# yabebalFantaye/MCEvidence

Hardware: AMD Instinct MI355X
Metric: knn_queries_per_sec (higher is better)
Workload: dtype f16 filter + f64 refine (exact f64 results)

## Files before the change

### mcevidence_amd/csrc/capi_search.hpp

```cpp
#pragma once
namespace {

double ln_unit_ball(int d) { return 0.5 * d * std::log(M_PI) - std::lgamma(1.0 + 0.5 * d); }

hipError_t launch_sym_merge(int KCAP, double* pd, int* pi, int64_t nq_pad, const mce::SymParams& sym, int qb_lo, int qb_hi, hipStream_t st, int stride = 1)
{
    const int nb = qb_hi > qb_lo ? (qb_hi - qb_lo + stride - 1) / stride : 0;
    if (nb <= 0) return hipSuccess;
    const dim3 g((unsigned)nb), b(mce::kSymMergeThreads);
    static_assert(mce::kSymMergeThreads == mce::f16_qpb(4), "one merge block per query block");
    switch (KCAP) {
        case 4: hipLaunchKernelGGL(mce::sym_merge_kernel<4>, g, b, 0, st, pd, pi, nq_pad, sym.bucket_cnt, sym.bucket_flag, sym.bucket, sym.cap, qb_lo, stride); break;
        case 8: hipLaunchKernelGGL(mce::sym_merge_kernel<8>, g, b, 0, st, pd, pi, nq_pad, sym.bucket_cnt, sym.bucket_flag, sym.bucket, sym.cap, qb_lo, stride); break;
        case 12: hipLaunchKernelGGL(mce::sym_merge_kernel<12>, g, b, 0, st, pd, pi, nq_pad, sym.bucket_cnt, sym.bucket_flag, sym.bucket, sym.cap, qb_lo, stride); break;
        default: hipLaunchKernelGGL(mce::sym_merge_kernel<16>, g, b, 0, st, pd, pi, nq_pad, sym.bucket_cnt, sym.bucket_flag, sym.bucket, sym.cap, qb_lo, stride); break;
    }
    return hipGetLastError();
}

struct KernelBracket {
    bool on = false; hipStream_t st = nullptr;
    hipError_t begin() const
    {
        if (!on) return hipSuccess;
// ... 307 lines not shown
        units = mce::panel_unit_count(g);
        for (int u = 0; g_prof_on && u < units; ++u) {
            int pp, aa, lo, hi;
            mce::panel_unit_decode(u, g, pp, aa);
            mce::panel_unit_tiles(pp, aa, g, lo, hi);
            tiles += hi - lo;
        }
    } else {
        const double tpb = mce::kHWaves * mce::kHQT, T = (double)((nr + 31) / 32);
        for (int b = 0; b < p.nqblk; ++b) tiles += std::min(tpb * (b + 1), T);
    }
    g_last_flops_main = tiles * 16.0 * 1024.0 * 32.0 * p.KST;
    return units;
}

int Search::symmetric()
{
    char* const sw = ws + p.off_sym;
    mce::KnnF16Args a = sym_args(p, ws, nr, d, K, self_exclude);
    const Tuning tun = read_tuning();
    const int seed_rows = tun.sym_seed_rows > 0 ? tun.sym_seed_rows : (p.KST == 1 ? 65536 : 32768) * (p.apo && p.nparts >= 4 ? 2 : 1);
    const int seed_share = tun.sym_seed_share;
    auto sym_seed_for = [&](int kk) {
        int cfg = mce::f16_seed_cfg(p.nchunk, p.CT, kk + a.self_exclude, seed_rows, seed_share, MCE_H_SEED_TG);
        for (int tg = MCE_H_SEED_TG / 2; cfg == 0 && tg >= 1; tg /= 2)
            cfg = mce::f16_seed_cfg(p.nchunk, p.CT, kk + a.self_exclude, seed_rows, seed_share, tg);
        if (cfg) cfg |= ((tun.sym_seed_mode >= 0 ? tun.sym_seed_mode : kSymSeedMode[p.KST]) & 3) << 28;
        return cfg;
    };
    const int qb_lo = p.nparts > 1 && !p.apo ? (int)((int64_t)p.nqblk * p.part / p.nparts) : 0;
    const int qb_hi = p.nparts > 1 && !p.apo ? (int)((int64_t)p.nqblk * (p.part + 1) / p.nparts) : p.nqblk;
    p.sym_qb_lo = qb_lo; p.sym_qb_hi = qb_hi;
    const bool panel_kernel = !tun.sym_kernel_f16 || p.nparts > 1 || p.twopass;
    mce::PanelGeom geom;
    geom.qb_lo = qb_lo; geom.qb_hi = qb_hi; geom.tpb = mce::kHWaves * mce::kHQT; geom.ct = p.CT; geom.tpp = a.sym.panel * p.CT; geom.sym_on = 1;
    geom.ntiles = (int)((nr + 31) / 32) + (int)(((nr + 31) / 32) & 1);
    const bool apo = p.apo && p.nparts > 1 && !p.twopass && panel_kernel;
    const bool chains1 = !apo && p.nparts == 1 && panel_kernel && !p.twopass && p.sym_nsplit > 1;
    if (apo) { geom.blk_first = p.part; geom.blk_stride = p.nparts; }
    if (apo || chains1) {
        const int pn = apo ? p.apo_panel : p.sym_panel;
        if (pn > 0 && (apo || tun.sym_panel <= 0)) { a.sym.panel = pn; geom.tpp = a.sym.panel * p.CT; }
        geom.nsplit = std::max(1, apo ? p.apo_nsplit : p.sym_nsplit);
        if (geom.nsplit > 1) {
            a.sym.done = reinterpret_cast<int*>(sw + p.sl.keys_b);
            MCE_HIP(mce::zero_async(a.sym.done, (size_t)p.nqblk * geom.nsplit * sizeof(int), st));
            if (!apo) {
                hipLaunchKernelGGL(mce::sym_chain_init_kernel, dim3((unsigned)p.nqblk), dim3(512), 0, st, pd, pi, p.nq_pad, p.KCAP, geom.nsplit, 0, 1);
                MCE_HIP(hipGetLastError());
            }
        }
    }
    const bool unit_table = apo || geom.nsplit > 1;
    const int npass = p.twopass ? 2 : 1;
    int seed_used = 0;
    for (int pass = 0; pass < npass; ++pass) {
        const bool lower = pass == 1;
        const int Kp = !p.twopass ? K : (lower ? K - 16 : 16);
        double* const pdp = pd + (lower ? list_set(p, 1) : 0);
        int* const pip = pi + (lower ? list_set(p, 1) : 0);
        if (lower) {
            MCE_HIP(mce::zero_async(a.sym.bucket_cnt, (size_t)3 * p.nqblk * sizeof(int), st));
            a.sym.slot_stride = p.KCAP;
        }
        a.ksel = lower ? K : Kp;
        a.seed_cfg = sym_seed_for(a.ksel);
        a.part_d = pdp; a.part_i = pip;
        a.qblk0 = qb_lo;
        a.nqblk_run = qb_hi - qb_lo;
        if (apo) {
            a.qblk0 = p.part; a.qblk_stride = p.nparts; a.nqblk_run = mce::apo_rank_count(p.nqblk, p.part, p.nparts);
        }
        if (a.nqblk_run > 0 && phase != 2) MCE_HIP((lower ? p.vh->launch_sym_pre32 : p.vh->launch_sym_pre)(a, st));
        a.qblk0 = 0; a.qblk_stride = 1; a.nqblk_run = 0;
        if (phase == 1) return MCE_OK;
        if (pass == 0) seed_used = a.seed_cfg;
        a.seed_cfg = 0;
        a.ksel = Kp;
        a.lo_d = lower ? pd : nullptr; a.lo_i = lower ? pi : nullptr;
        if (pass == 0) MCE_HIP(kb.begin());
        if (panel_kernel) {
            mce::PanelArgs pa;
            pa.Yh = static_cast<const _Float16*>(a.Yh); pa.Xh = static_cast<const _Float16*>(a.Xh); pa.qinfo = a.qinfo; pa.params = a.params;
            pa.X = a.X; pa.Y = a.Y; pa.rperm = a.rperm;
            pa.part_d = pdp; pa.part_i = pip; pa.nq = nq; pa.nr = nr; pa.nq_pad = p.nq_pad; pa.self_offset = 0;
            pa.D = d; pa.ksel = Kp; pa.self_exclude = a.self_exclude; pa.spin_limit = tun.spin_limit;
            pa.sym = a.sym; pa.debug = tun.panel_debug; pa.geom = geom; pa.lo_d = a.lo_d; pa.lo_i = a.lo_i;
            if (unit_table) {
                const int nun = mce::panel_unit_count(geom);
                if ((size_t)nun * sizeof(mce::PanelUnit) > (size_t)p.nq_pad * sizeof(int)) return fail(MCE_ERR_INVALID, "symmetric sweep: %d units do not fit the table", nun);
                mce::PanelUnit* tab = reinterpret_cast<mce::PanelUnit*>(sw + p.sl.vals_a);
                if (nun > 0) {
                    hipLaunchKernelGGL(mce::panel_unit_table_kernel, dim3((unsigned)((nun + 255) / 256)), dim3(256), 0, st, geom, nun, tab);
                    MCE_HIP(hipGetLastError());
                }
                pa.units = tab;
            }
            MCE_HIP((lower ? p.vh->launch_panel_lower : p.vh->launch_panel)(pa, st));
        } else {
            MCE_HIP(p.vh->launch_sym(a, st));
        }
        if (pass == 0) MCE_HIP(kb.end());
        if (apo) break;
        MCE_HIP((lower ? p.vh->launch_sym_repair_lower : p.vh->launch_sym_repair)(a, st));
        if (geom.nsplit > 1) {
            hipLaunchKernelGGL(mce::sym_chain_clear_kernel, dim3((unsigned)p.nqblk), dim3(512), 0, st, a.sym.bucket_flag, pdp, pip, p.nq_pad, p.KCAP, geom.nsplit, 0, 1);
            MCE_HIP(hipGetLastError());
        }
        MCE_HIP(launch_sym_merge(p.KCAP, pdp, pip, p.nq_pad, a.sym, qb_lo, qb_hi, st));
    }
    p.sym_active = true;
    p.L = geom.nsplit > 1 ? geom.nsplit : npass;
    const int sym_units = sym_units_and_flops(p, geom, panel_kernel, nr, a.sym.panel);
    g_last_flops_all = g_last_flops_main + (double)(seed_used & 0xffff) * p.CT * (double)(qb_hi - qb_lo) * 16.0 * 1024.0 * 32.0 * p.KST;
    snprintf(g_last_kernel, sizeof(g_last_kernel), "%s symmetric%s%s%s grid=%d block=%d lds=%zu qt=%d ct=%d panel=%d seed=%dx%d/%d bucket=%d", p.vh->name, panel_kernel ? " panel-kernel" : "",
             p.twopass ? " two passes" : "", geom.blk_stride > 1 ? " pairs-once" : (geom.nsplit > 1 ? " chains" : ""), sym_units,
             mce::kHThreads, panel_kernel ? p.vh->lds_bytes_panel : p.vh->lds_bytes_sym, p.QT, p.CT, a.sym.panel, seed_used & 0xffff, (seed_used >> 16) & 0xfff, (seed_used >> 28) & 3, p.sl.cap);
    return MCE_OK;
}

int Search::f16_sweep(const F16Search& f)
{
    mce::KnnF16Args a = f16_args(p, ws, f.sX, nq, f.sY, nr, d, K, self_exclude, self_offset);
    auto seed_cfg = [&](int ksel) { return sweep_seed_cfg(p.nchunk / p.rsplit, p.CT, ksel + a.self_exclude); };
    MCE_HIP(kb.begin());
    if (p.twopass) {
        a.ksel = 16;
        a.seed_cfg = seed_cfg(16);
        MCE_HIP(p.vh->launch(a, st));
        a.lo_d = pd; a.lo_i = pi;
        a.part_d = pd + list_set(p, p.rsplit); a.part_i = pi + list_set(p, p.rsplit);
        a.ksel = K - 16;
        a.seed_cfg = 0;
        MCE_HIP(p.vh->launch_lower(a, st));
    } else {
        a.seed_cfg = seed_cfg(K);
        if (p.wide_ok) MCE_HIP(p.vh->launch_wide(a, st));
        else MCE_HIP(p.vh->launch(a, st));
    }
    MCE_HIP(kb.end());
    const int seed_first = p.twopass ? seed_cfg(16) : a.seed_cfg;
    g_last_flops_main = (double)p.nqblk * ((double)p.nchunk + (double)(seed_first & 0xffff) * p.rsplit) * p.CT * 16.0 * 1024.0 * 32.0 * p.KST +
                        (p.twopass ? (double)p.nqblk * (double)p.nchunk * p.CT * 16.0 * 1024.0 * 32.0 * p.KST : 0.0);
    g_last_flops_all = g_last_flops_main;
    char seed_txt[48] = "";
    if (seed_first) snprintf(seed_txt, sizeof(seed_txt), " seed=%dx%d", seed_first & 0xffff, seed_first >> 16);
    const bool wide = p.wide_ok && !p.twopass;
    snprintf(g_last_kernel, sizeof(g_last_kernel), "%s grid=%d block=%d lds=%zu qt=%d ct=%d rsplit=%d%s%s%s", p.vh->name,
             (wide ? p.nqblk / 2 : p.nqblk) * p.rsplit, mce::kHThreads, wide ? p.vh->lds_bytes_wide : p.vh->lds_bytes, wide ? 2 * p.QT : p.QT, p.CT, p.rsplit,
             p.twopass ? " two passes" : "", seed_txt, wide ? " wide" : "");
    return MCE_OK;
}

int Search::fp64()
{
    const int threads = 256;
    double* yf = reinterpret_cast<double*>(ws + p.off_yf);
    hipLaunchKernelGGL(mce::pack_refs_kernel, dim3((unsigned)((p.nrow_pad + threads - 1) / threads)), dim3(threads), 0, st, dY, nr,
                       (int)d, p.KS, p.nrow_pad, center, yf);
    MCE_HIP(hipGetLastError());
    mce::KnnArgs a;
    a.Yf = yf; a.nchunk_total = p.nchunk; a.rsplit = p.rsplit; a.X = dX; a.center = center; a.nq = nq; a.D = d;
    a.nq_pad = p.nq_pad; a.nqblk = p.nqblk; a.self_exclude = self_exclude; a.self_offset = self_offset;
    a.ksel = p.ksel > K ? p.ksel : K;
    a.part_d = pd; a.part_i = pi;
    MCE_HIP(kb.begin());
    MCE_HIP(p.v->launch(a, st));
// ... 98 lines not shown
```

### mcevidence_amd/csrc/knn_panel.hpp

```cpp
#pragma once
#include "knn_f16.hpp"

namespace mce {

struct PanelArgs {
    const _Float16* Yh;
    const _Float16* Xh;
    const double* qinfo;
    const double* params;
    const double* X;
    const double* Y;
    const int* rperm;
    double* part_d;
    int* part_i;
    int64_t nq, nr, nq_pad, self_offset;
    int D, ksel, self_exclude, spin_limit;
    int debug;
    SymParams sym;
    PanelGeom geom;
    const PanelUnit* units = nullptr;
    const double* lo_d = nullptr;
    const int* lo_i = nullptr;
};

#ifndef MCE_PANEL_STATS
#define MCE_PANEL_STATS 0
#endif
#ifndef MCE_PANEL_NPASS
#define MCE_PANEL_NPASS 3
#endif
#ifndef MCE_PANEL_STAGE_KB
#define MCE_PANEL_STAGE_KB MCE_H_STAGE_KB
#endif
#ifndef MCE_PANEL_QUEUE
#define MCE_PANEL_QUEUE MCE_H_QUEUE
#endif
#ifndef MCE_PANEL_TRIGGER
#define MCE_PANEL_TRIGGER 192
#endif
#ifndef MCE_PANEL_ABL
#define MCE_PANEL_ABL 0
#endif

__host__ __device__ constexpr int panel_chunk_tiles(int KST) { return MCE_PANEL_STAGE_KB / KST / 2 * 2; }
constexpr int kPanelQueue = MCE_PANEL_QUEUE;
__host__ __device__ constexpr size_t panel_lds_bytes(int KST)
{
    return (size_t)2 * panel_chunk_tiles(KST) * KST * 1024
           + (size_t)kHWaves * kPanelQueue * 16
           + (size_t)kHWaves * kHQT * 32 * 4 + 128
           + (size_t)kHWaves * kHQT * 32 * 4
           + (size_t)kHWaves * panel_chunk_tiles(KST) * kHQT * 4;
}

template <class T> __device__ __forceinline__ const __attribute__((address_space(1))) T* gptr(const T* p)
{
    return (const __attribute__((address_space(1))) T*)p;
}
template <class T> __device__ __forceinline__ __attribute__((address_space(1))) T* gptr_w(T* p)
{
    return (__attribute__((address_space(1))) T*)p;
}

__device__ __forceinline__ float vmaxf(float a, float b)
{
    float r;
    asm("v_max_f32 %0, %1, %2" : "=v"(r) : "v"(a), "v"(b));
    return r;
}

template <int KST, int KCAP, bool LOWER = false>
__global__ __launch_bounds__(kHThreads, 2) void knn_panel_kernel(PanelArgs args_by_value)
{
    static_assert(kHQT == 2 && kHNL == 1, "8 waves x 2 query tiles, one list per owner lane");
    constexpr int QT = 2;
    constexpr int QPW = 64;
    constexpr int QPB = kHWaves * QPW;
    constexpr int TPB = QPB / 32;
    constexpr int CT = panel_chunk_tiles(KST);
    constexpr int CHUNK_BYTES = CT * KST * 1024;
    constexpr int VPT = CHUNK_BYTES / 16 / kHThreads;
    static_assert(CHUNK_BYTES % (16 * kHThreads) == 0 && CT % 2 == 0, "chunk geometry");
    constexpr int QN = kPanelQueue;
    (void)args_by_value;
// ... 100 lines not shown
            } else if (lane == 0) {
                gptr_w(a->sym.bucket_flag)[qblk] = 1;
            }
        }
    }

    v8h b[QT][KST];
    float G[QT], cR[QT];
    unsigned lanew[QT];
    const int k_last = MCE_ARGS()->ksel - 1;
    {
        const ArgsPtr a = MCE_ARGS();
        const auto Xh = gptr(a->Xh);
#pragma unroll
        for (int qt = 0; qt < QT; ++qt) {
            const int64_t q = qwave0 + qt * 32 + (lane & 31);
#pragma unroll
            for (int ks = 0; ks < KST; ++ks)
                b[qt][ks] = *(const __attribute__((address_space(1))) v8h*)(Xh + q * (int64_t)(16 * KST) + 16 * ks + 8 * (lane >> 5));
            lanew[qt] = ((unsigned)(qt * 32 + (lane & 31)) << kHRelBits) | (unsigned)(4 * (lane >> 5));
            cR[qt] = -__builtin_huge_valf();
            G[qt] = -__builtin_huge_valf();
        }
    }
    double gq_a[QT], gq_c[QT], own_a = 0.0, s2c, rowc;
    {
        const ArgsPtr a = MCE_ARGS();
        const auto params = gptr(a->params);
        const auto qinfo = gptr(a->qinfo);
        const double p_scale = params[HP_SCALE], p_ey = params[HP_EY], p_ym = params[HP_YHATMAX], p_rho = params[HP_RHO];
        s2c = p_scale * p_scale;
        rowc = f16_row_const(p_ym);
#pragma unroll
        for (int qt = 0; qt < QT; ++qt) {
            const int64_t q = qwave0 + qt * 32 + (lane & 31);
            gq_a[qt] = 0.0;
            gq_c[qt] = -INF;
            if (q < a->nq && MCE_PANEL_ABL != 1) {
                const F16GateTerms t = f16_gate_terms(qinfo[2 * q], qinfo[2 * q + 1], p_ey, p_ym, p_rho, KST);
                gq_a[qt] = t.a;
                gq_c[qt] = t.c;
            }
        }
        {
            const int64_t q = qwave0 + lane;
            if (q < a->nq) own_a = f16_gate_a(qinfo[2 * q], p_ey, KST);
        }
    }
    auto gate_of = [&](double thr, int qt) __attribute__((always_inline)) -> float { return f16_gate(thr, s2c, gq_a[qt], gq_c[qt]); };
    auto own_row_gate = [&](double thr) __attribute__((always_inline)) -> float { return f16_row_gate(thr, s2c, own_a, rowc); };
    {
        const ArgsPtr a = MCE_ARGS();
        const int64_t q = qwave0 + lane;
        double t0 = INF;
        if (sym_on) t0 = __longlong_as_double((long long)__hip_atomic_load(gptr(a->sym.thr) + q, __ATOMIC_RELAXED, __HIP_MEMORY_SCOPE_AGENT));
        else if (a->sym.thr) t0 = __longlong_as_double((long long)gptr(a->sym.thr)[q]);
        seed_thr = t0;
        double tl = own_d[KCAP - 1];
#pragma unroll
        for (int k = 0; k < KCAP - 1; ++k) tl = (k == k_last) ? own_d[k] : tl;
        t0 = fmin(t0, tl);
        sthr[lane] = __double2float_ru(t0);
#pragma unroll
        for (int qt = 0; qt < QT; ++qt) G[qt] = gate_of(__shfl(t0, qt * 32 + (lane & 31), 64), qt);
        if (sym_on) {
#pragma unroll
            for (int qt = 0; qt < QT; ++qt) cR[qt] = gq_c[qt] > -INF ? f16_round_up(gq_c[qt]) : -__builtin_huge_valf();
        }
    }

    const int dbg_flags = MCE_ARGS()->debug;
    const int qlimit_gate = (dbg_flags & 8) ? -1 : QN - 64;
    int qcount = 0;
    int nredo = 0;

    auto drain = [&]() __attribute__((always_inline)) {
#if MCE_PANEL_STATS
        const long long t_d0 = clock64();
        st_drains += 1; st_enq += qcount;
#endif
        const ArgsPtr a = MCE_ARGS();
        const auto X = gptr(a->X);
        const auto Y = gptr(a->Y);
        const int D = a->D;
        const int64_t nq = a->nq, nr = a->nr;
        const int self_exclude = a->self_exclude;
        const int64_t self_offset = a->self_offset;
        const auto rperm = gptr(a->rperm);
        {
            const int sub = lane & 7;
            constexpr int NPASS = KST > 2 ? 1 : MCE_PANEL_NPASS;
            constexpr int EPL = KST > 2 ? 8 : 4;
            for (int b0 = 0; b0 < qcount; b0 += NPASS * 8) {
                int qlp[NPASS], ep[NPASS];
                bool okp[NPASS];
                const __attribute__((address_space(1))) double* xp[NPASS];
                const __attribute__((address_space(1))) double* yp[NPASS];
#pragma unroll
                for (int u = 0; u < NPASS; ++u) {
                    const int e = b0 + u * 8 + (lane >> 3);
                    ep[u] = e;
                    int ql = 0, j = 0;
                    const bool valid = e < qcount;
                    if (valid) {
                        const unsigned ent = (unsigned)wq[e];
                        ql = (int)(ent >> kHRelBits);
                        j = (int)(ent & ((1u << kHSymRowBits) - 1u));
                    }
                    qlp[u] = ql;
                    const int64_t q = qwave0 + ql;
                    okp[u] = valid && j < nr && q < nq && !(self_exclude && (int64_t)j == self_offset + q);
                    xp[u] = X + (okp[u] ? q : 0) * (int64_t)D;
                    yp[u] = Y + (okp[u] ? (int64_t)j : 0) * D;
                }
                double xv[NPASS][EPL], yv[NPASS][EPL];
#pragma unroll
                for (int u = 0; u < NPASS; ++u)
#pragma unroll
                    for (int v = 0; v < EPL; ++v) {
                        const int iv = (sub + 8 * v < D) ? sub + 8 * v : (sub < D ? sub : D - 1);
                        xv[u][v] = xp[u][iv];
                        yv[u][v] = yp[u][iv];
                    }
#pragma unroll
                for (int u = 0; u < NPASS; ++u) {
                    double a0 = 0.0;
#pragma unroll
                    for (int v = 0; v < EPL; ++v) {
                        const double t = (sub + 8 * v < D) ? xv[u][v] - yv[u][v] : 0.0;
                        a0 = fma(t, t, a0);
                    }
                    a0 += __shfl_xor(a0, 1, 64);
                    a0 += __shfl_xor(a0, 2, 64);
                    a0 += __shfl_xor(a0, 4, 64);
                    if (sub == 0 && ep[u] < qcount) {
                        wqd[ep[u]] = okp[u] ? a0 : -1.0;
                        bool col = okp[u] && !(a0 > (double)sthr[qlp[u]]);
                        if constexpr (LOWER) {
                            if (col) {
                                const int64_t o = (int64_t)(KCAP - 1) * a->nq_pad + qwave0 + qlp[u];
                                const double ld = gptr(a->lo_d)[o];
                                const int li = gptr(a->lo_i)[o];
                                const int jr = (int)((unsigned)wq[ep[u]] & ((1u << kHSymRowBits) - 1u));
                                const int jc = rperm ? rperm[jr] : jr;
                                col = a0 > ld || (a0 == ld && jc > li);
                            }
                        }
                        if (col) wnx[ep[u]] = atomicExch(&whead[qlp[u]], ep[u]);
                    }
                }
            }
        }
        __builtin_amdgcn_fence(__ATOMIC_ACQ_REL, "wavefront");
#if MCE_PANEL_STATS
        const long long t_dA = clock64();
        st_tA += t_dA - t_d0;
#endif
        {
            const auto sp_thr = gptr_w(a->sym.thr);
            const auto sp_rrow = gptr_w(a->sym.rrow);
            const auto sp_rtile = gptr_w(a->sym.rtile);
            const auto sp_slots = gptr_w(a->sym.slots);
            const auto sp_bucket_cnt = gptr_w(a->sym.bucket_cnt);
            const auto sp_bucket_flag = gptr_w(a->sym.bucket_flag);
            const auto sp_bucket = gptr_w(a->sym.bucket);
            const int sp_cap = a->sym.cap;
            const int ksel = a->ksel;
            auto row_gate = [&](double thr, int row) { return f16_row_gate_of(thr, gptr(a->qinfo)[2 * (int64_t)row], a->params, KST); };
            for (int e0 = 0; e0 < qcount; e0 += 64) {
                const int e = e0 + lane;
                const bool valid = e < qcount;
                const unsigned ent = valid ? (unsigned)wq[e] : 0u;
                const int ql = (int)(ent >> kHRelBits);
                const int j = (int)(ent & ((1u << kHSymRowBits) - 1u));
                const bool rowflag = (ent >> kHSymRowBits) & 1u;
                const double d2 = valid ? wqd[e] : -1.0;
                const bool ok = valid && d2 >= 0.0;
                const int oj = ok ? (rperm ? rperm[j] : j) : -1;
                bool rs = ok && rowflag;
                if (rs) {
                    const int jb = j / QPB;
                    rs = d2 <= __longlong_as_double((long long)__hip_atomic_load(sp_thr + j, __ATOMIC_RELAXED, __HIP_MEMORY_SCOPE_AGENT));
                    if constexpr (LOWER) {
                        if (rs) {
                            const int64_t o = (int64_t)(KCAP - 1) * a->nq_pad + j;
                            const double ld = gptr(a->lo_d)[o];
                            const int li = gptr(a->lo_i)[o];
                            const int sc = rperm ? rperm[qwave0 + ql] : (int)(qwave0 + ql);
                            rs = d2 > ld || (d2 == ld && sc > li);
                        }
                    }
                    if (rs) rs = sym_slot_insert<KCAP>(sp_slots, sp_thr, sp_rrow, sp_rtile, ksel, j, d2, row_gate);
                    if (rs) {
                        const int slot = __hip_atomic_fetch_add(sp_bucket_cnt + jb, 1, __ATOMIC_RELAXED, __HIP_MEMORY_SCOPE_AGENT);
                        if ((unsigned)slot < (unsigned)sp_cap) {
                            const auto en = sp_bucket + ((int64_t)jb * sp_cap + slot);
                            en->d2 = d2;
                            en->src = rperm ? rperm[qwave0 + ql] : (int)(qwave0 + ql);
                            en->row = j;
                        } else {
                            sp_bucket_flag[jb] = 1;
                        }
                    }
                }
                if (valid) wq[e] = oj;
            }
        }
        __builtin_amdgcn_fence(__ATOMIC_ACQ_REL, "wavefront");
#if MCE_PANEL_STATS
        const long long t_dR = clock64();
        st_tR += t_dR - t_dA;
#endif
        {
            int cur = whead[lane];
            whead[lane] = -1;
            while (__any(cur >= 0)) {
                const bool on = cur >= 0;
                const int ce = on ? cur : 0;
                const double d2 = on ? wqd[ce] : INF;
                const int j = wq[ce];
                cur = on ? wnx[ce] : -1;
                list_insert<KCAP>(own_d, own_i, d2, j);
            }
        }
        qcount = 0;
        double thr_own = own_d[KCAP - 1];
#pragma unroll
        for (int k = 0; k < KCAP - 1; ++k) thr_own = (k == k_last) ? own_d[k] : thr_own;
        thr_own = fmin(thr_own, seed_thr);
        if (sym_on) {
            const auto sp_thr = gptr_w(a->sym.thr);
            const auto sp_rrow = gptr_w(a->sym.rrow);
            const auto sp_rtile = gptr_w(a->sym.rtile);
            const int64_t q = qwave0 + lane;
            double t = thr_own;
            float R = 0.0f;
            if (q < nq) {
                if (t < INF) {
                    const unsigned long long mb = (unsigned long long)__double_as_longlong(t);
                    const unsigned rb = __float_as_uint(own_row_gate(t));
                    const unsigned long long ob = __hip_atomic_fetch_min(sp_thr + q, mb, __ATOMIC_RELAXED, __HIP_MEMORY_SCOPE_AGENT);
                    const unsigned orb = __hip_atomic_fetch_min(sp_rrow + q, rb, __ATOMIC_RELAXED, __HIP_MEMORY_SCOPE_AGENT);
                    t = fmin(t, __longlong_as_double((long long)ob));
                    R = __uint_as_float(rb < orb ? rb : orb);
                } else {
                    t = __longlong_as_double((long long)__hip_atomic_load(sp_thr + q, __ATOMIC_RELAXED, __HIP_MEMORY_SCOPE_AGENT));
                    const unsigned rb = __float_as_uint(own_row_gate(t));
                    const unsigned orb = __hip_atomic_fetch_min(sp_rrow + q, rb, __ATOMIC_RELAXED, __HIP_MEMORY_SCOPE_AGENT);
                    R = __uint_as_float(rb < orb ? rb : orb);
                }
            }
            thr_own = t;
            seed_thr = t;
            float m = R;
#pragma unroll
            for (int o = 16; o >= 1; o >>= 1) m = fmaxf(m, __shfl_xor(m, o, 64));
            if ((lane & 31) == 0) __hip_atomic_store(sp_rtile + ((qwave0 + lane) >> 5), m, __ATOMIC_RELAXED, __HIP_MEMORY_SCOPE_AGENT);
        }
        sthr[lane] = __double2float_ru(thr_own);
#pragma unroll
        for (int qt = 0; qt < QT; ++qt) G[qt] = gate_of(__shfl(thr_own, qt * 32 + (lane & 31), 64), qt);
#if MCE_PANEL_STATS
        st_tD += clock64() - t_d0;
#endif
    };

    auto event = [&](const v16f& c, const float (&l1)[5], const int qt, const float gq, const bool rowflag, const int jb0, const unsigned todo, const int qlimit) __attribute__((always_inline)) -> unsigned {
        return f16_event<true>(c, l1, lanew[qt], gq, rowflag, jb0, todo, qlimit, wq, qcount);
    };

    const auto Yh_bytes = (const __attribute__((address_space(1))) char*)MCE_ARGS()->Yh;
    auto stage_async = [&](int64_t c, int buf) { f16_stage_chunk<VPT>(Yh_bytes + c * (int64_t)CHUNK_BYTES, stage0 + buf * CHUNK_BYTES, tid, wave); };
    auto load_a = [&](const char* lp, v8h (&a)[KST]) { f16_load_a<KST>(lp, a); };
    auto mfma_first = [&](const v8h (&a)[KST], v16f (&acc)[QT]) __attribute__((always_inline)) {
#pragma unroll
        for (int qt = 0; qt < QT; ++qt) {
            v16f z = {0.f, 0.f, 0.f, 0.f, 0.f, 0.f, 0.f, 0.f, 0.f, 0.f, 0.f, 0.f, 0.f, 0.f, 0.f, 0.f};
            acc[qt] = __builtin_amdgcn_mfma_f32_32x32x16_f16(a[0], b[qt][0], z, 0, 0, 0);
        }
    };
    auto mfma_rest = [&](const v8h (&a)[KST], v16f (&acc)[QT]) __attribute__((always_inline)) {
#pragma unroll
        for (int ks = 1; ks < KST; ++ks)
#pragma unroll
            for (int qt = 0; qt < QT; ++qt) acc[qt] = __builtin_amdgcn_mfma_f32_32x32x16_f16(a[ks], b[qt][ks], acc[qt], 0, 0, 0);
    };
#if defined(__HIP_DEVICE_COMPILE__)
#define MCE_ORDER(GATED_, NEXT_) asm volatile("" : "+v"(GATED_[0]), "+v"(GATED_[1]), "+v"(NEXT_[0]), "+v"(NEXT_[1]))
// ... 188 lines not shown
```

### mcevidence_amd/csrc/prune.hip

```cpp
#include "prune.hpp"
#include "zero_fill.hpp"

#include <cstdlib>
#include <cstring>

#include <rocprim/device/device_radix_sort.hpp>

#include <algorithm>

namespace mce {

namespace {

constexpr int kThreads = 256;

size_t align_up(size_t x, size_t a) { return (x + a - 1) / a * a; }

constexpr int kCoordBits = 24;
constexpr int kMinCoordBits32 = 18;
constexpr int kAlign = 64;
constexpr int kAlignLevels = 6;

int top_tree_levels(int64_t n_units)
{
    const int64_t groups = (n_units + kAlign - 1) / kAlign;
    int L = 0;
    while (((int64_t)1 << L) < groups) ++L;
    return L;
}

template <class Key>
__global__ __launch_bounds__(kThreads) void kd_key_kernel(const int* __restrict__ perm_in, int64_t n, int64_t n_pad, int unit_rows,
                                                          int n_units, int top_levels, int level, const float* __restrict__ Cf, int d, int dim,
                                                          int cbits, Key* __restrict__ keys, int* __restrict__ vals, int64_t pos0 = 0, int64_t pos1 = -1)
{
    const int64_t pos = pos0 + (int64_t)blockIdx.x * kThreads + threadIdx.x;
    if (pos >= (pos1 < 0 ? n_pad : pos1)) return;
    const int row = perm_in ? perm_in[pos] : (pos < n ? (int)pos : -1);
    const int u = (int)(pos / unit_rows);
    const int cu = u / kAlign;
    int clo = 0, chi = (n_units + kAlign - 1) / kAlign;
    unsigned id = 0;
    int l = 0;
    for (; l < level && l < top_levels; ++l) {
        if (chi - clo > 1) {
            const int mid = (clo + chi) >> 1;
            if (cu < mid) { chi = mid; id = 2 * id; }
            else { clo = mid; id = 2 * id + 1; }
        } else {
            id = 2 * id;
        }
    }
    for (int half = kAlign >> 1; l < level; ++l, half >>= 1) id = 2 * id + ((u & half) ? 1u : 0u);
    unsigned b = 0xFFFFFFFFu;
    if (row >= 0) {
        const float c = Cf[(int64_t)dim * n + row];
        b = __float_as_uint(c);
        b = (b & 0x80000000u) ? ~b : (b | 0x80000000u);
        if (b == 0xFFFFFFFFu) b = 0xFFFFFFFEu;
        b >>= (32 - cbits);
        if (b == (0xFFFFFFFFu >> (32 - cbits))) b -= 1u;
    } else {
        b >>= (32 - cbits);
    }
    keys[pos] = (Key)(((Key)id << cbits) | (Key)b);
    vals[pos] = row;
}

constexpr int kGroupRows = kAlign * kPruneTileRows;
constexpr int kBottomSlots = kGroupRows + kGroupRows / 32;
__device__ __forceinline__ int bslot(int i) { return i + (i >> 5); }
__global__ __launch_bounds__(kThreads) void kd_bottom_kernel(int* __restrict__ perm, int64_t n, int64_t n_pad, int top_levels, const float* __restrict__ Cf, int d,
                                                             int64_t group0 = 0)
{
    static_assert(kGroupRows == 8 * kThreads, "eight slots per thread");
    __shared__ unsigned long long key[kBottomSlots];
    __shared__ int val[2][kGroupRows];
    const int64_t base = (group0 + (int64_t)blockIdx.x) * kGroupRows;
    const int m = (int)(n_pad - base < kGroupRows ? n_pad - base : kGroupRows);
    for (int i = threadIdx.x; i < kGroupRows; i += kThreads) val[0][i] = i < m ? perm[base + i] : -2;
    __syncthreads();
    int cur = 0;
    for (int l = 0; l < kAlignLevels; ++l) {
        const int dim = (top_levels + l) % d;
// ... 485 lines not shown
    hipLaunchKernelGGL(group_box_kernel, blocks_for((int64_t)nqblk * d), dim3(kThreads), 0, st, out.tbox_q, same_set ? ntile_r : ntile_q, d,
                       qpb / kPruneTileRows, nqblk, box_q);
    if ((e = hipGetLastError()) != hipSuccess) return e;
    static_assert(kBandKeys % kThreads == 0 && kPruneMaxDim * 2 <= kThreads, "chunk_list_kernel geometry");
    if (nchunk <= kListStage) {
        static bool attr_set[16] = {};
        int dev = 0;
        (void)hipGetDevice(&dev);
        if (dev >= 16 || !attr_set[dev]) {
            e = hipFuncSetAttribute(reinterpret_cast<const void*>(chunk_list_kernel), hipFuncAttributeMaxDynamicSharedMemorySize, (int)chunk_list_lds_bytes(kListStage));
            if (e != hipSuccess) return e;
            if (dev < 16) attr_set[dev] = true;
        }
        hipLaunchKernelGGL(chunk_list_kernel, dim3((unsigned)nqblk), dim3(kThreads), chunk_list_lds_bytes((int)nchunk), st, box_q, box_r, (int)nchunk, d, list_d_b, list_c_b);
    } else {
        hipLaunchKernelGGL(chunk_list_big_kernel, dim3((unsigned)nqblk), dim3(kThreads), 0, st, box_q, box_r, (int)nchunk, d, list_d_b, list_c_b);
    }
    if ((e = hipGetLastError()) != hipSuccess) return e;
    {
        float* bkey_a = reinterpret_cast<float*>(ws + L.bkey_a);
        float* bkey_b = reinterpret_cast<float*>(ws + L.bkey_b);
        int* bval_a = reinterpret_cast<int*>(ws + L.bval_a);
        int* border = reinterpret_cast<int*>(ws + L.border);
        const int nwaves = nqblk * kPruneWavesPerBlock;
        const int tpw = qpb / kPruneTileRows / kPruneWavesPerBlock;
        hipLaunchKernelGGL(wave_cost_kernel, dim3((unsigned)((nwaves + kThreads - 1) / kThreads)), dim3(kThreads), 0, st, out.tbox_q, nwaves, tpw,
                           same_set ? ntile_r : ntile_q, d, bkey_a, bval_a);
        if ((e = hipGetLastError()) != hipSuccess) return e;
        size_t tb2 = L.tmp_bytes;
        e = rocprim::radix_sort_pairs_desc(tmp, tb2, (const float*)bkey_a, bkey_b, (const int*)bval_a, border, (size_t)nwaves, 0u, 32u, st);
        if (e != hipSuccess) return e;
        out.border = border;
    }
    out.Ys = Ys;
    out.rperm = perm_r;
    out.clist = list_c_b;
    out.cdist = list_d_b;
    return hipSuccess;
}

namespace {

constexpr int kNormRows = 256;
__global__ __launch_bounds__(kNormRows) void norm_key_kernel(const double* __restrict__ Y, int64_t n, int64_t n_pad, int d,
                                                             const double* __restrict__ center, unsigned* __restrict__ keys,
                                                             int* __restrict__ vals)
{
    extern __shared__ double tile[];
    const int64_t r0 = (int64_t)blockIdx.x * kNormRows;
    const int64_t rows = n - r0 < kNormRows ? (n - r0 > 0 ? n - r0 : 0) : kNormRows;
    const int ld = d + 1;
    for (int64_t e = threadIdx.x; e < rows * d; e += kNormRows) {
        const int r = (int)(e / d), c = (int)(e - (int64_t)r * d);
        tile[r * ld + c] = Y[r0 * d + e] - center[c];
    }
    __syncthreads();
    const int64_t pos = r0 + threadIdx.x;
    if (pos >= n_pad) return;
    unsigned k = 0xFFFFFFFFu;
    if (pos < n) {
        double s = 0.0;
        for (int i = 0; i < d; ++i) {
            const double t = tile[threadIdx.x * ld + i];
            s = fma(t, t, s);
        }
        k = __float_as_uint((float)s);
        if (k > 0xFFFFFFFEu || s != s) k = 0xFFFFFFFEu;
    }
    keys[pos] = k;
    vals[pos] = pos < n ? (int)pos : -1;
}

}

int sym_layout(int64_t n, int64_t n_pad, int nqblk, int d, int kcap, int qpb, int per_row, SymLayout& L)
{
    size_t off = 0;
    auto take = [&](size_t bytes) { const size_t o = off; off = align_up(off + bytes, 256); return o; };
    L.perm = take((size_t)n_pad * 4);
    L.keys_a = take((size_t)n_pad * 4);
    L.keys_b = take((size_t)n_pad * 4);
    L.vals_a = take((size_t)n_pad * 4);
    L.Ys = take((size_t)n * d * 8);
    L.thr = take((size_t)n_pad * 8);
    L.rrow = take((size_t)n_pad * 4);
    L.rtile = take((size_t)(n_pad / 32) * 4);
    L.slots = take((size_t)n_pad * kcap * 8);
    L.bucket_cnt = take((size_t)nqblk * 4 * 3);
    L.bucket_flag = L.bucket_cnt + (size_t)nqblk * 4;
    L.done = L.bucket_flag + (size_t)nqblk * 4;
    L.cap = per_row * qpb;
    L.bucket = take((size_t)nqblk * L.cap * 16);
    L.tmp_bytes = sort_pairs_tmp_bytes<unsigned>(n_pad, 32u);
    L.tmp = take(L.tmp_bytes);
    L.total = off;
    return 0;
}

hipError_t sym_prepare(const double* dY, int64_t n, int d, const double* center, int64_t n_pad, char* ws, const SymLayout& L, hipStream_t st)
{
    int* perm = reinterpret_cast<int*>(ws + L.perm);
    unsigned* keys_a = reinterpret_cast<unsigned*>(ws + L.keys_a);
    unsigned* keys_b = reinterpret_cast<unsigned*>(ws + L.keys_b);
    int* vals_a = reinterpret_cast<int*>(ws + L.vals_a);
    double* Ys = reinterpret_cast<double*>(ws + L.Ys);
    const unsigned blocks = (unsigned)((n_pad + kNormRows - 1) / kNormRows);
    hipLaunchKernelGGL(norm_key_kernel, dim3(blocks), dim3(kNormRows), (size_t)kNormRows * (d + 1) * sizeof(double), st, dY, n, n_pad, d, center,
                       keys_a, vals_a);
    hipError_t e = hipGetLastError();
    if (e != hipSuccess) return e;
    e = sort_pairs(ws + L.tmp, L.tmp_bytes, (const unsigned*)keys_a, keys_b, (const int*)vals_a, perm, n_pad, 32u, st);
    if (e != hipSuccess) return e;
    hipLaunchKernelGGL(gather_rows_kernel, dim3((unsigned)((n * d + kThreads - 1) / kThreads)), dim3(kThreads), 0, st, dY, perm, n, d, Ys);
    if ((e = hipGetLastError()) != hipSuccess) return e;
    e = zero_async(ws + L.bucket_cnt, (size_t)3 * (L.bucket_flag - L.bucket_cnt), st);
    return e;
}

}
```

### mcevidence_amd/csrc/prune.hpp

```cpp
#pragma once
#include <hip/hip_runtime.h>
#include <stddef.h>
#include <stdint.h>

namespace mce {

constexpr int kPruneTileRows = 32;
constexpr int kPruneMaxDim = 15;
constexpr int64_t kPruneMaxPairs = (int64_t)1 << 30;
constexpr int kPruneWavesPerBlock = 8;

struct PruneLayout {
    size_t perm_r = 0, perm_q = 0;
    size_t keys_a = 0, keys_b = 0;
    size_t vals_b = 0;
    size_t Ys = 0, Xs = 0;
    size_t cf32 = 0;
    size_t tbox_r = 0, tbox_q = 0;
    size_t tboxT_r = 0;
    size_t box_r = 0, box_q = 0;
    size_t bkey_a = 0, bkey_b = 0, bval_a = 0, border = 0;
    size_t list_d_b = 0, list_c_b = 0;
    size_t tmp = 0, tmp_bytes = 0;
    size_t total = 0;
};

int prune_layout(int64_t nq, int64_t nq_pad, int nqblk, int64_t nr, int64_t nr_pad, int64_t nchunk, int d, PruneLayout& L);

constexpr int kPruneBandMantissa = 5;
__host__ __device__ inline float prune_band_floor(float d2)
{
#if defined(__HIP_DEVICE_COMPILE__)
    return __uint_as_float(__float_as_uint(d2) & ~((1u << (23 - kPruneBandMantissa)) - 1u));
#else
    union { float f; unsigned u; } v; v.f = d2; v.u &= ~((1u << (23 - kPruneBandMantissa)) - 1u); return v.f;
#endif
}

struct PruneOut {
    const double* Xs = nullptr;
    const double* Ys = nullptr;
    const int* qperm = nullptr;
    const int* rperm = nullptr;
    const int* clist = nullptr;
    const float* cdist = nullptr;
    const float* tbox_r = nullptr;
    const float* tbox_q = nullptr;
    const float* cbox_r = nullptr;
    const int* border = nullptr;
};

hipError_t prune_prepare(const double* dX, int64_t nq, const double* dY, int64_t nr, int d, bool same_set, int qpb,
                         int chunk_rows, int64_t nq_pad, int nqblk, int64_t nr_pad, int64_t nchunk, char* ws,
                         const PruneLayout& L, hipStream_t st, PruneOut& out, bool perm_ready = false);
hipError_t prune_prepare_part(const double* dY, int64_t nr, int d, int64_t nr_pad, char* ws, const PruneLayout& L, int part, int nparts,
                              hipStream_t st, int64_t& seg_lo, int64_t& seg_hi);

struct SymLayout {
    size_t perm = 0;
    size_t keys_a = 0, keys_b = 0;
    size_t vals_a = 0;
    size_t Ys = 0;
    size_t thr = 0;
    size_t rrow = 0;
    size_t rtile = 0;
    size_t slots = 0;
    size_t bucket_cnt = 0, bucket_flag = 0, done = 0;
    size_t bucket = 0;
    size_t tmp = 0, tmp_bytes = 0;
    size_t total = 0;
    int cap = 0;
};
int sym_layout(int64_t n, int64_t n_pad, int nqblk, int d, int kcap, int qpb, int per_row, SymLayout& L);
hipError_t sym_prepare(const double* dY, int64_t n, int d, const double* center, int64_t n_pad, char* ws, const SymLayout& L,
                       hipStream_t st);

}
```

Before: 26.86 million.

## Refine from padded lane-interleaved f64 image and batch survivor threshold loads

Measured after the change: 27.06 million, median of 6. Within noise of the previous version (+0.8%).

```diff
diff --git a/mcevidence_amd/csrc/capi_search.hpp b/mcevidence_amd/csrc/capi_search.hpp
--- a/mcevidence_amd/csrc/capi_search.hpp
+++ b/mcevidence_amd/csrc/capi_search.hpp
@@ -413,7 +413,8 @@
         if (panel_kernel) {
             mce::PanelArgs pa;
             pa.Yh = static_cast<const _Float16*>(a.Yh); pa.Xh = static_cast<const _Float16*>(a.Xh); pa.qinfo = a.qinfo; pa.params = a.params;
-            pa.X = a.X; pa.Y = a.Y; pa.rperm = a.rperm;
+            if (p.sl.img_pitch != mce::refine_pitch(p.KST)) return fail(MCE_ERR_INVALID, "symmetric sweep: refine image of pitch %d, the kernel reads %d", p.sl.img_pitch, mce::refine_pitch(p.KST));
+            pa.X = pa.Y = reinterpret_cast<const double*>(sw + p.sl.Yimg); pa.rperm = a.rperm;
             pa.part_d = pdp; pa.part_i = pip; pa.nq = nq; pa.nr = nr; pa.nq_pad = p.nq_pad; pa.self_offset = 0;
             pa.D = d; pa.ksel = Kp; pa.self_exclude = a.self_exclude; pa.spin_limit = tun.spin_limit;
             pa.sym = a.sym; pa.debug = tun.panel_debug; pa.geom = geom; pa.lo_d = a.lo_d; pa.lo_i = a.lo_i;
diff --git a/mcevidence_amd/csrc/knn_panel.hpp b/mcevidence_amd/csrc/knn_panel.hpp
--- a/mcevidence_amd/csrc/knn_panel.hpp
+++ b/mcevidence_amd/csrc/knn_panel.hpp
@@ -1,5 +1,6 @@
 #pragma once
 #include "knn_f16.hpp"
+#include "refine_image.hpp"
 
 namespace mce {
 
@@ -266,23 +267,30 @@
         const ArgsPtr a = MCE_ARGS();
         const auto X = gptr(a->X);
         const auto Y = gptr(a->Y);
-        const int D = a->D;
         const int64_t nq = a->nq, nr = a->nr;
         const int self_exclude = a->self_exclude;
         const int64_t self_offset = a->self_offset;
         const auto rperm = gptr(a->rperm);
+        int dl = lane;
+#if defined(__HIP_DEVICE_COMPILE__)
+        asm volatile("" : "+v"(dl));
+#endif
         {
-            const int sub = lane & 7;
+            typedef double v2d __attribute__((ext_vector_type(2)));
+            typedef const __attribute__((address_space(1))) v2d* RowPtr;
+            const int sub = dl & 7;
             constexpr int NPASS = KST > 2 ? 1 : MCE_PANEL_NPASS;
-            constexpr int EPL = KST > 2 ? 8 : 4;
+            constexpr int EPL = refine_epl(KST);
+            constexpr int PITCH = refine_pitch(KST);
+            const auto Xl = X + EPL * sub;
+            const auto Yl = Y + EPL * sub;
             for (int b0 = 0; b0 < qcount; b0 += NPASS * 8) {
                 int qlp[NPASS], ep[NPASS];
                 bool okp[NPASS];
-                const __attribute__((address_space(1))) double* xp[NPASS];
-                const __attribute__((address_space(1))) double* yp[NPASS];
+                RowPtr xp[NPASS], yp[NPASS];
 #pragma unroll
                 for (int u = 0; u < NPASS; ++u) {
-                    const int e = b0 + u * 8 + (lane >> 3);
+                    const int e = b0 + u * 8 + (dl >> 3);
                     ep[u] = e;
                     int ql = 0, j = 0;
                     const bool valid = e < qcount;
@@ -294,24 +302,24 @@
                     qlp[u] = ql;
                     const int64_t q = qwave0 + ql;
                     okp[u] = valid && j < nr && q < nq && !(self_exclude && (int64_t)j == self_offset + q);
-                    xp[u] = X + (okp[u] ? q : 0) * (int64_t)D;
-                    yp[u] = Y + (okp[u] ? (int64_t)j : 0) * D;
-                }
-                double xv[NPASS][EPL], yv[NPASS][EPL];
+                    static_assert(kHSymRowBits + 6 <= 32, "an image row's element index fits 32 bits");
+                    xp[u] = (RowPtr)(Xl + (size_t)((unsigned)(okp[u] ? (int)q : 0) * (unsigned)PITCH));
+                    yp[u] = (RowPtr)(Yl + (size_t)((unsigned)(okp[u] ? j : 0) * (unsigned)PITCH));
+                }
+                v2d xv[NPASS][EPL / 2], yv[NPASS][EPL / 2];
 #pragma unroll
                 for (int u = 0; u < NPASS; ++u)
 #pragma unroll
-                    for (int v = 0; v < EPL; ++v) {
-                        const int iv = (sub + 8 * v < D) ? sub + 8 * v : (sub < D ? sub : D - 1);
-                        xv[u][v] = xp[u][iv];
-                        yv[u][v] = yp[u][iv];
+                    for (int v = 0; v < EPL / 2; ++v) {
+                        xv[u][v] = xp[u][v];
+                        yv[u][v] = yp[u][v];
                     }
 #pragma unroll
                 for (int u = 0; u < NPASS; ++u) {
                     double a0 = 0.0;
 #pragma unroll
                     for (int v = 0; v < EPL; ++v) {
-                        const double t = (sub + 8 * v < D) ? xv[u][v] - yv[u][v] : 0.0;
+                        const double t = xv[u][v / 2][v & 1] - yv[u][v / 2][v & 1];
                         a0 = fma(t, t, a0);
                     }
                     a0 += __shfl_xor(a0, 1, 64);
@@ -351,31 +359,64 @@
             const int sp_cap = a->sym.cap;
             const int ksel = a->ksel;
             auto row_gate = [&](double thr, int row) { return f16_row_gate_of(thr, gptr(a->qinfo)[2 * (int64_t)row], a->params, KST); };
-            for (int e0 = 0; e0 < qcount; e0 += 64) {
-                const int e = e0 + lane;
-                const bool valid = e < qcount;
-                const unsigned ent = valid ? (unsigned)wq[e] : 0u;
-                const int ql = (int)(ent >> kHRelBits);
-                const int j = (int)(ent & ((1u << kHSymRowBits) - 1u));
-                const bool rowflag = (ent >> kHSymRowBits) & 1u;
-                const double d2 = valid ? wqd[e] : -1.0;
-                const bool ok = valid && d2 >= 0.0;
-                const int oj = ok ? (rperm ? rperm[j] : j) : -1;
-                bool rs = ok && rowflag;
-                if (rs) {
-                    const int jb = j / QPB;
-                    rs = d2 <= __longlong_as_double((long long)__hip_atomic_load(sp_thr + j, __ATOMIC_RELAXED, __HIP_MEMORY_SCOPE_AGENT));
-                    if constexpr (LOWER) {
-                        if (rs) {
+            constexpr int NB = (QN + 63) / 64;
+            unsigned surv = 0u;
+            {
+                const auto thr_rd = sp_thr ? (const __attribute__((address_space(1))) unsigned long long*)sp_thr
+                                           : (const __attribute__((address_space(1))) unsigned long long*)gptr(a->params);
+                unsigned long long thb[NB];
+                int ojb[NB];
+                double ldb[LOWER ? NB : 1];
+                int lib[LOWER ? NB : 1], scb[LOWER ? NB : 1];
+#pragma unroll
+                for (int bi = 0; bi < NB; ++bi) {
+                    if (bi * 64 < qcount) {
+                        const int e = bi * 64 + dl;
+                        const bool valid = e < qcount;
+                        const unsigned ent = valid ? (unsigned)wq[e] : 0u;
+                        const bool ok = valid && wqd[e] >= 0.0;
+                        const int j = ok ? (int)(ent & ((1u << kHSymRowBits) - 1u)) : 0;
+                        const int jt = ((ent >> kHSymRowBits) & 1u) ? j : 0;
+                        thb[bi] = __hip_atomic_load(thr_rd + jt, __ATOMIC_RELAXED, __HIP_MEMORY_SCOPE_AGENT);
+                        ojb[bi] = rperm ? rperm[j] : j;
+                        if constexpr (LOWER) {
                             const int64_t o = (int64_t)(KCAP - 1) * a->nq_pad + j;
-                            const double ld = gptr(a->lo_d)[o];
-                            const int li = gptr(a->lo_i)[o];
-                            const int sc = rperm ? rperm[qwave0 + ql] : (int)(qwave0 + ql);
-                            rs = d2 > ld || (d2 == ld && sc > li);
+                            const int ql = ok ? (int)(ent >> kHRelBits) : 0;
+                            ldb[bi] = gptr(a->lo_d)[o];
+                            lib[bi] = gptr(a->lo_i)[o];
+                            scb[bi] = rperm ? rperm[qwave0 + ql] : (int)(qwave0 + ql);
                         }
                     }
-                    if (rs) rs = sym_slot_insert<KCAP>(sp_slots, sp_thr, sp_rrow, sp_rtile, ksel, j, d2, row_gate);
-                    if (rs) {
+                }
+#pragma unroll
+                for (int bi = 0; bi < NB; ++bi) {
+                    if (bi * 64 < qcount) {
+                        const int e = bi * 64 + dl;
+                        const bool valid = e < qcount;
+                        const unsigned ent = valid ? (unsigned)wq[e] : 0u;
+                        const double d2 = valid ? wqd[e] : -1.0;
+                        const bool ok = valid && d2 >= 0.0;
+                        const bool rowflag = (ent >> kHSymRowBits) & 1u;
+                        bool rs = ok && rowflag && d2 <= __longlong_as_double((long long)thb[bi]);
+                        if constexpr (LOWER) {
+                            rs = rs && (d2 > ldb[bi] || (d2 == ldb[bi] && scb[bi] > lib[bi]));
+                        }
+                        if (rs) surv |= 1u << bi;
+                        else if (valid) wq[e] = ok ? ojb[bi] : -1;
+                    }
+                }
+            }
+            while (__any(surv != 0u)) {
+                if (surv != 0u) {
+                    const int e = (__builtin_ctz(surv) << 6) + dl;
+                    surv &= surv - 1u;
+                    const unsigned ent = (unsigned)wq[e];
+                    const int ql = (int)(ent >> kHRelBits);
+                    const int j = (int)(ent & ((1u << kHSymRowBits) - 1u));
+                    const double d2 = wqd[e];
+                    const int jb = j / QPB;
+                    const int oj = rperm ? rperm[j] : j;
+                    if (sym_slot_insert<KCAP>(sp_slots, sp_thr, sp_rrow, sp_rtile, ksel, j, d2, row_gate)) {
                         const int slot = __hip_atomic_fetch_add(sp_bucket_cnt + jb, 1, __ATOMIC_RELAXED, __HIP_MEMORY_SCOPE_AGENT);
                         if ((unsigned)slot < (unsigned)sp_cap) {
                             const auto en = sp_bucket + ((int64_t)jb * sp_cap + slot);
@@ -386,8 +427,8 @@
                             sp_bucket_flag[jb] = 1;
                         }
                     }
-                }
-                if (valid) wq[e] = oj;
+                    wq[e] = oj;
+                }
             }
         }
         __builtin_amdgcn_fence(__ATOMIC_ACQ_REL, "wavefront");
diff --git a/mcevidence_amd/csrc/prune.hip b/mcevidence_amd/csrc/prune.hip
--- a/mcevidence_amd/csrc/prune.hip
+++ b/mcevidence_amd/csrc/prune.hip
@@ -1,5 +1,6 @@
 #include "prune.hpp"
 #include "zero_fill.hpp"
+#include "refine_image.hpp"
 
 #include <cstdlib>
 #include <cstring>
@@ -651,6 +652,8 @@
     L.keys_b = take((size_t)n_pad * 4);
     L.vals_a = take((size_t)n_pad * 4);
     L.Ys = take((size_t)n * d * 8);
+    L.img_pitch = refine_pitch_dim(d);
+    L.Yimg = take((size_t)n_pad * L.img_pitch * 8);
     L.thr = take((size_t)n_pad * 8);
     L.rrow = take((size_t)n_pad * 4);
     L.rtile = take((size_t)(n_pad / 32) * 4);
@@ -680,7 +683,13 @@
     if (e != hipSuccess) return e;
     e = sort_pairs(ws + L.tmp, L.tmp_bytes, (const unsigned*)keys_a, keys_b, (const int*)vals_a, perm, n_pad, 32u, st);
     if (e != hipSuccess) return e;
-    hipLaunchKernelGGL(gather_rows_kernel, dim3((unsigned)((n * d + kThreads - 1) / kThreads)), dim3(kThreads), 0, st, dY, perm, n, d, Ys);
+    if (L.img_pitch) {
+        double* Yimg = reinterpret_cast<double*>(ws + L.Yimg);
+        hipLaunchKernelGGL(gather_rows_image_kernel, dim3((unsigned)((n * L.img_pitch + 255) / 256)), dim3(256), 0, st, dY, (const int*)perm, n, d,
+                           L.img_pitch / 8, Ys, Yimg);
+    } else {
+        hipLaunchKernelGGL(gather_rows_kernel, dim3((unsigned)((n * d + kThreads - 1) / kThreads)), dim3(kThreads), 0, st, dY, perm, n, d, Ys);
+    }
     if ((e = hipGetLastError()) != hipSuccess) return e;
     e = zero_async(ws + L.bucket_cnt, (size_t)3 * (L.bucket_flag - L.bucket_cnt), st);
     return e;
diff --git a/mcevidence_amd/csrc/prune.hpp b/mcevidence_amd/csrc/prune.hpp
--- a/mcevidence_amd/csrc/prune.hpp
+++ b/mcevidence_amd/csrc/prune.hpp
@@ -61,6 +61,8 @@
     size_t keys_a = 0, keys_b = 0;
     size_t vals_a = 0;
     size_t Ys = 0;
+    size_t Yimg = 0;
+    int img_pitch = 0;
     size_t thr = 0;
     size_t rrow = 0;
     size_t rtile = 0;
diff --git a/mcevidence_amd/csrc/refine_image.hpp b/mcevidence_amd/csrc/refine_image.hpp
--- /dev/null
+++ b/mcevidence_amd/csrc/refine_image.hpp
@@ -0,0 +1,39 @@
+#pragma once
+#include <stdint.h>
+#if defined(__HIPCC__)
+#include <hip/hip_runtime.h>
+#endif
+
+namespace mce {
+
+#if defined(__HIPCC__)
+#define MCE_RI_HD __host__ __device__
+#else
+#define MCE_RI_HD
+#endif
+
+MCE_RI_HD constexpr int refine_epl(int KST) { return KST > 2 ? 8 : 4; }
+MCE_RI_HD constexpr int refine_pitch(int KST) { return 8 * refine_epl(KST); }
+MCE_RI_HD constexpr int refine_pitch_dim(int D) { return D < 1 || D > 63 ? 0 : (D < 32 ? 32 : 64); }
+
+#if defined(__HIPCC__)
+static __global__ __launch_bounds__(256) void gather_rows_image_kernel(const double* __restrict__ P, const int* __restrict__ perm, int64_t n, int d,
+                                                                        int epl, double* __restrict__ out, double* __restrict__ img)
+{
+    const int lg = epl == 8 ? 6 : 5;
+    const int64_t e = (int64_t)blockIdx.x * 256 + threadIdx.x;
+    if (e >= (n << lg)) return;
+    const int64_t pos = e >> lg;
+    const int p = (int)(e - (pos << lg));
+    const int sub = epl == 8 ? p >> 3 : p >> 2;
+    const int c = sub + 8 * (p - sub * epl);
+    double v = 0.0;
+    if (c < d) {
+        v = P[(perm ? (int64_t)perm[pos] : pos) * d + c];
+        if (out) out[pos * d + c] = v;
+    }
+    img[e] = v;
+}
+#endif
+
+}
```
